# google/telluride_decoding

Hardware: AMD Instinct MI355X
Metric: TRF-fit samples/sec (higher is better)
Workload: dtype f32 (every product as 3 float16 products of a 2-piece split on the f16 MFMA, f32 accumulate, f64 slab sums; f64 solve)

## Files before the change

telluride_decoding_amd/csrc/lag_targets.hip:

```cpp
#include <cstdlib>
#include <cstring>

#include "lag_common.h"

namespace {

constexpr int kWaveStrip = 512;

template <int E, int NI>
__global__ __launch_bounds__(kThreads) void lagcov_wave_kernel(LagParams p, double* __restrict__ part64,
                                                              double* __restrict__ csum,
                                                              double* __restrict__ ysum) {
  constexpr int P = 32;
  constexpr int NY = NI > 0 ? NI : 1;
  constexpr int kRowsMax = ((kWaveStrip + 2 * E - 2) / E) * E;
  __shared__ float ylds[kThreads / 64][kRowsMax * NY];
  const int tid = threadIdx.x, lane = tid & 63;
  const int wave = __builtin_amdgcn_readfirstlane(tid >> 6);
  long long id = blockIdx.x * (long long)(kThreads / 64) + wave;
  if (id >= (long long)p.n_work * p.n_cbt) return;
  const int cbt = (int)(id % p.n_cbt);
  const int wi = (int)(id / p.n_cbt);
  const LagWork w = p.works[wi];
  const int len = (int)(w.u_end - w.u_begin);
// ... 206 lines not shown
      if (!kHalf) slab[(size_t)k * p.ca_pad * p.cb_pad + c0 + 1] = big1[r];
    }
  }
  if (g == 0 && csum) {
    csum[(size_t)slab_i * p.cb_pad + c0] = cs0;
    if (!kHalf) csum[(size_t)slab_i * p.cb_pad + c0 + 1] = cs1;
  }
}

template <bool kVec2, bool kHalf = false>
__global__ __launch_bounds__(kThreads) void lagcov_targets_mfma_kernel(LagParams p,
                                                                       double* __restrict__ part64,
                                                                       double* csum, double* ysum,
                                                                       unsigned* maxtab) {
  constexpr int E = 32, P = kTgtPrefetch, kPad = 32, kRowsBody = 2 * kTgtBody;
  constexpr int kBodiesMax = (kTgtStrip + E - 1 + kRowsBody - 1) / kRowsBody;
  __shared__ float ya[kPad + kBodiesMax * kRowsBody];
  __shared__ double comb[3][16][64];
  const int tid = threadIdx.x, lane = tid & 63;
  const int wave = __builtin_amdgcn_readfirstlane(tid >> 6);
  const int n_win = p.n_groups;
  const int slot = (int)(blockIdx.x >> 3);
  const int item = (slot / n_win) * 8 + (int)(blockIdx.x & 7);
  if (item >= p.n_work * p.n_cbt) return;
  const int cbt = item % p.n_cbt;
  const int wi = item / p.n_cbt;
  const LagWork w = p.works[wi];
  const int e_lo = 32 * (slot % n_win);
  p.e_min += e_lo;
  if (e_lo) { csum = nullptr; ysum = nullptr; maxtab = nullptr; }
  const TgtStrip ts = tgt_strip(p, w);
  const int slab_i = wi;
  tgt_stage_targets(p, w, ts.len, ts.n_body, kPad, ya, tid);
  __syncthreads();
  if (cbt == 0 && ysum && wave == 0) {
    double sy = 0.0;
    for (int t = lane; t < ts.len; t += 64) sy += (double)ya[kPad + t];
#pragma unroll
    for (int off = 32; off > 0; off >>= 1) sy += __shfl_down(sy, off, 64);
    if (lane == 0) ysum[slab_i] = sy;
  }

  const int n = lane & 31, g = lane >> 5;
  const int c0 = kHalf ? cbt * 64 + n : cbt * 64 + 2 * n;
  const bool ok0 = c0 < p.cb, ok1 = !kHalf && c0 + 1 < p.cb;
  const int off0 = ok0 ? c0 : 0, off1 = ok1 ? c0 + 1 : off0;
  int b0 = wave, nb = 0;
  while (b0 < ts.n_body && !tgt_body_fast(ts, b0)) b0 += 4;
  for (int b = b0; b < ts.n_body && tgt_body_fast(ts, b); b += 4) ++nb;

  f32x16 acc0, acc1;
  double big0[16], big1[16];
#pragma unroll
  for (int r = 0; r < 16; ++r) { acc0[r] = 0.f; acc1[r] = 0.f; big0[r] = 0.0; big1[r] = 0.0; }
  double cs0 = 0.0, cs1 = 0.0;
  float mx0 = 0.f, mx1 = 0.f;
  const float* yp = ya + kPad + g - n;
  if (nb > 0) {
    float xr[P][2];
    auto load_step = [&](const float* bp, int s, float& x0, float& x1) {
      if (kHalf) {
        x0 = bp[s * 2 * ts.ldb32]; x1 = 0.f;
      } else if (kVec2) {
        const float2 v = *reinterpret_cast<const float2*>(bp + s * 2 * ts.ldb32);
        x0 = v.x; x1 = v.y;
      } else {
        x0 = bp[s * 2 * ts.ldb32]; x1 = bp[s * 2 * ts.ldb32 + off1 - off0];
      }
    };
    {
      const float* bp = ts.strip + (b0 * kRowsBody + g - ts.r_lo) * ts.ldb32 + off0;
#pragma unroll
      for (int k = 0; k < P; ++k) load_step(bp, k, xr[k][0], xr[k][1]);
    }
    for (int it = 0; it < nb; ++it) {
      const int b = b0 + 4 * it;
      const float* bp = ts.strip + ((b + 4) * kRowsBody + g - ts.r_lo) * ts.ldb32 + off0;
      float c0s = 0.f, c1s = 0.f;
#pragma unroll
      for (int s = 0; s < kTgtBody; ++s) {
        const float x0 = xr[s % P][0], x1 = xr[s % P][1];
        c0s += x0; c1s += x1;
        mx0 = fmaxf(mx0, fabsf(x0)); mx1 = fmaxf(mx1, fabsf(x1));
        const float a = yp[(b * kTgtBody + s) * 2];
        acc0 = __builtin_amdgcn_mfma_f32_32x32x2f32(a, x0, acc0, 0, 0, 0);
        if (!kHalf) acc1 = __builtin_amdgcn_mfma_f32_32x32x2f32(a, x1, acc1, 0, 0, 0);
        load_step(bp, s, xr[s % P][0], xr[s % P][1]);
      }
      cs0 += (double)c0s;
      cs1 += (double)c1s;
#pragma unroll
      for (int r = 0; r < 16; ++r) {
        big0[r] += (double)acc0[r]; acc0[r] = 0.f;
        if (!kHalf) { big1[r] += (double)acc1[r]; acc1[r] = 0.f; }
      }
    }
  }
  for (int b = wave; b < ts.n_body; b += 4) {
    if (tgt_body_fast(ts, b)) continue;
    float c0s = 0.f, c1s = 0.f;
    float xe[kTgtBody][2];
#pragma unroll
    for (int s = 0; s < kTgtBody; ++s) {
      const int r = (b * kTgtBody + s) * 2 + g;
      const int rc = min(max(r, ts.r_lo), ts.r_hi) - ts.r_lo;
      const float* rowp = ts.strip + rc * ts.ldb32;
      if (kHalf) {
        xe[s][0] = rowp[off0]; xe[s][1] = 0.f;
      } else if (kVec2) {
        const float2 v = *reinterpret_cast<const float2*>(rowp + off0);
        xe[s][0] = v.x; xe[s][1] = v.y;
      } else {
        xe[s][0] = rowp[off0]; xe[s][1] = rowp[off1];
      }
    }
#pragma unroll
    for (int s = 0; s < kTgtBody; ++s) {
      const int r = (b * kTgtBody + s) * 2 + g;
      const float m = (r >= ts.r_lo && (long long)r <= ts.last) ? 1.f : 0.f;
      const float x0 = xe[s][0] * m, x1 = xe[s][1] * m;
      mx0 = fmaxf(mx0, fabsf(x0)); mx1 = fmaxf(mx1, fabsf(x1));
      const float in = (r >= ts.t_lo && r < ts.t_hi) ? 1.f : 0.f;
      c0s = fmaf(in, x0, c0s); c1s = fmaf(in, x1, c1s);
      const float a = yp[(b * kTgtBody + s) * 2];
      acc0 = __builtin_amdgcn_mfma_f32_32x32x2f32(a, x0, acc0, 0, 0, 0);
      if (!kHalf) acc1 = __builtin_amdgcn_mfma_f32_32x32x2f32(a, x1, acc1, 0, 0, 0);
    }
    cs0 += (double)c0s;
    cs1 += (double)c1s;
#pragma unroll
    for (int r = 0; r < 16; ++r) {
      big0[r] += (double)acc0[r]; acc0[r] = 0.f;
      if (!kHalf) { big1[r] += (double)acc1[r]; acc1[r] = 0.f; }
    }
  }
  tgt_combine_store<kHalf>(p, part64, csum, maxtab, comb, slab_i, e_lo, c0, ok0, ok1, big0, big1, cs0, cs1,
                           mx0, mx1);
}

constexpr int kTgtBodiesMax = (kTgtStrip + 31 + 31) / 32;
constexpr int kTgtImage = (32 + kTgtBodiesMax * 32) / 2 + 8;

__device__ __forceinline__ int tgt_scale_exp(unsigned max_bits) {
  if (max_bits == 0 || td_chan_not_finite(max_bits)) return 0;
  return 15 - __builtin_amdgcn_frexp_expf(__uint_as_float(max_bits));
}

__device__ __forceinline__ void tgt_split2(float x0, float x1, unsigned& h, unsigned& l) {
  h = td_pack_f16(x0, x1);
  const td_f16x2 hv = __builtin_bit_cast(td_f16x2, h);
  l = td_pack_f16(__builtin_fmaf((float)hv[0], -1.f, x0), __builtin_fmaf((float)hv[1], -1.f, x1));
}

template <class Refill>
__device__ __forceinline__ void tgt_split_body(float (&x)[kTgtBody][2], unsigned mb0, unsigned mb1,
                                               const unsigned* ah, const unsigned* al, int ky, bool y_bad,
                                               double (&big0)[16], double (&big1)[16], Refill refill) {
  mb0 = max(mb0, (unsigned)__shfl_xor((int)mb0, 32, 64));
  mb1 = max(mb1, (unsigned)__shfl_xor((int)mb1, 32, 64));
  const int k0 = tgt_scale_exp(mb0), k1 = tgt_scale_exp(mb1);
  td_u32x4 h0[2], l0[2], h1[2], l1[2];
#pragma unroll
  for (int ks = 0; ks < 2; ++ks)
#pragma unroll
    for (int j = 0; j < 4; ++j) {
      const int s = 8 * ks + 2 * j;
      unsigned h, l;
      tgt_split2(ldexpf(x[s][0], k0), ldexpf(x[s + 1][0], k0), h, l);
      h0[ks][j] = h; l0[ks][j] = l;
      tgt_split2(ldexpf(x[s][1], k1), ldexpf(x[s + 1][1], k1), h, l);
      h1[ks][j] = h; l1[ks][j] = l;
      refill(s);
      refill(s + 1);
    }
  __builtin_amdgcn_sched_barrier(0);
  td_f32x16 acc0, acc1;
#pragma unroll
  for (int r = 0; r < 16; ++r) { acc0[r] = 0.f; acc1[r] = 0.f; }
#pragma unroll
  for (int ks = 0; ks < 2; ++ks) {
    const td_u32x4 yh = {ah[4 * ks], ah[4 * ks + 1], ah[4 * ks + 2], ah[4 * ks + 3]};
    const td_u32x4 yl = {al[4 * ks], al[4 * ks + 1], al[4 * ks + 2], al[4 * ks + 3]};
    acc0 = td_mfma_f16(yl, h0[ks], acc0);
    acc1 = td_mfma_f16(yl, h1[ks], acc1);
    acc0 = td_mfma_f16(yh, l0[ks], acc0);
    acc1 = td_mfma_f16(yh, l1[ks], acc1);
    acc0 = td_mfma_f16(yh, h0[ks], acc0);
    acc1 = td_mfma_f16(yh, h1[ks], acc1);
  }
  const double nan = __hiloint2double(0x7ff80000, 0);
  const double f0 = (y_bad || td_chan_not_finite(mb0)) ? nan : __hiloint2double((1023 - k0 - ky) << 20, 0);
  const double f1 = (y_bad || td_chan_not_finite(mb1)) ? nan : __hiloint2double((1023 - k1 - ky) << 20, 0);
#pragma unroll
  for (int r = 0; r < 16; ++r) {
    big0[r] = fma((double)acc0[r], f0, big0[r]);
    big1[r] = fma((double)acc1[r], f1, big1[r]);
  }
}

__global__ __launch_bounds__(kThreads, 2) void lagcov_targets_split_kernel(LagParams p,
                                                                           double* __restrict__ part64,
                                                                           double* csum, double* ysum,
                                                                           unsigned* maxtab) {
  constexpr int kPad = 32, kRowsBody = 2 * kTgtBody;
  __shared__ float ya[kPad + kTgtBodiesMax * kRowsBody];
  __shared__ __attribute__((aligned(16))) _Float16 yimg[2][2][2][kTgtImage];
  __shared__ double comb[3][16][64];
  __shared__ unsigned ymax_w[kThreads / 64];
  const int tid = threadIdx.x, lane = tid & 63;
  const int wave = __builtin_amdgcn_readfirstlane(tid >> 6);
  const int item = (int)blockIdx.x;
  if (item >= p.n_work * p.n_cbt) return;
  const int cbt = item % p.n_cbt;
  const int wi = item / p.n_cbt;
  const LagWork w = p.works[wi];
  const TgtStrip ts = tgt_strip(p, w);
  const int n = lane & 31, g = lane >> 5;
  const int c0 = cbt * 64 + 2 * n;
  const bool ok0 = c0 < p.cb, ok1 = c0 + 1 < p.cb;
  const int off0 = ok0 ? c0 : 0;
  const int dg = g - n;
  const unsigned* ah = reinterpret_cast<const unsigned*>(&yimg[0][dg & 1][(dg >> 1) & 1][0]) + 8 + (dg >> 2);
  const unsigned* al = reinterpret_cast<const unsigned*>(&yimg[1][dg & 1][(dg >> 1) & 1][0]) + 8 + (dg >> 2);
  int b0 = wave, nb = 0;
  while (b0 < ts.n_body && !tgt_body_fast(ts, b0)) b0 += 4;
  for (int b = b0; b < ts.n_body && tgt_body_fast(ts, b); b += 4) ++nb;

  const long long rows_here = ts.last - ts.r_lo + 1;
  const long long rows_need = (long long)ts.n_body * kRowsBody;
  const unsigned buf_bytes =
      nb > 0 ? (unsigned)(((rows_here < rows_need ? rows_here : rows_need) - 1) * ts.ldb32 + p.cb) * 4u : 0u;
  const __amdgpu_buffer_rsrc_t rs =
      __builtin_amdgcn_make_buffer_rsrc(const_cast<float*>(ts.strip), 0, buf_bytes, 0x00020000);
  const unsigned voff = (unsigned)(g * ts.ldb32 + off0) * 4u;
  float xa[kTgtBody][2], xb[kTgtBody][2];
  auto load_step = [&](float (&xr)[kTgtBody][2], unsigned body_off, int s) {
    const td_f32x2 v = __builtin_bit_cast(
        td_f32x2, __builtin_amdgcn_raw_buffer_load_b64(rs, voff, body_off + (unsigned)(s * 2 * ts.ldb32) * 4u, 0));
    xr[s][0] = v[0]; xr[s][1] = v[1];
  };
  const int b_last = b0 + 4 * (nb - 1);
  auto body_off = [&](int b) { return (unsigned)(((b < b_last ? b : b_last) * kRowsBody - ts.r_lo) * ts.ldb32) * 4u; };
  if (nb > 0) {
    const unsigned bo0 = body_off(b0), bo1 = body_off(b0 + 4);
#pragma unroll
    for (int s = 0; s < kTgtBody; ++s) load_step(xa, bo0, s);
#pragma unroll
    for (int s = 0; s < kTgtBody; ++s) load_step(xb, bo1, s);
  }
  const int n_y = kPad + ts.n_body * kRowsBody;
  tgt_stage_targets(p, w, ts.len, ts.n_body, kPad, ya, tid);
  __syncthreads();
  {
    unsigned ym = 0u;
    for (int t = tid; t < n_y; t += kThreads) ym = max(ym, __float_as_uint(ya[t]) & 0x7fffffffu);
#pragma unroll
    for (int off = 32; off > 0; off >>= 1) ym = max(ym, (unsigned)__shfl_xor((int)ym, off, 64));
    if (lane == 0) ymax_w[wave] = ym;
  }
  if (cbt == 0 && ysum && wave == 0) {
    double sy = 0.0;
    for (int t = lane; t < ts.len; t += 64) sy += (double)ya[kPad + t];
#pragma unroll
    for (int off = 32; off > 0; off >>= 1) sy += __shfl_down(sy, off, 64);
    if (lane == 0) ysum[wi] = sy;
  }
  __syncthreads();
  const unsigned ymax = max(max(ymax_w[0], ymax_w[1]), max(ymax_w[2], ymax_w[3]));
  const bool y_bad = td_chan_not_finite(ymax);
  const int ky = tgt_scale_exp(ymax);
  for (int t = tid; t < n_y / 2; t += kThreads) {
#pragma unroll
    for (int q = 0; q < 2; ++q) {
      const float v = ldexpf(ya[2 * t + q], ky);
      const _Float16 hv = (_Float16)v;
      const _Float16 lv = (_Float16)(v - (float)hv);
      yimg[0][q][0][t] = hv;
      yimg[1][q][0][t] = lv;
      if (t > 0) { yimg[0][q][1][t - 1] = hv; yimg[1][q][1][t - 1] = lv; }
    }
  }
  __syncthreads();

  double big0[16], big1[16];
#pragma unroll
  for (int r = 0; r < 16; ++r) { big0[r] = 0.0; big1[r] = 0.0; }
  double cs0 = 0.0, cs1 = 0.0;
  float mx0 = 0.f, mx1 = 0.f;
  if (nb > 0) {
    auto pass = [&](float (&xr)[kTgtBody][2], int b) {
      const unsigned bo = body_off(b + 8);
      float c0s = 0.f, c1s = 0.f, m0 = 0.f, m1 = 0.f;
#pragma unroll
      for (int s = 0; s < kTgtBody; ++s) {
        c0s += xr[s][0]; c1s += xr[s][1];
        m0 = fmaxf(m0, fabsf(xr[s][0])); m1 = fmaxf(m1, fabsf(xr[s][1]));
      }
      cs0 += (double)c0s;
      cs1 += (double)c1s;
      mx0 = fmaxf(mx0, m0); mx1 = fmaxf(mx1, m1);
      const unsigned mb0 = fabsf(c0s) <= 3.402823466e38f ? __float_as_uint(m0) : 0x7fc00000u;
      const unsigned mb1 = fabsf(c1s) <= 3.402823466e38f ? __float_as_uint(m1) : 0x7fc00000u;
      tgt_split_body(xr, mb0, mb1, ah + 8 * b, al + 8 * b, ky, y_bad, big0, big1,
                     [&](int s) { load_step(xr, bo, s); });
    };
    for (int it = 0; it + 1 < nb; it += 2) {
      pass(xa, b0 + 4 * it);
      pass(xb, b0 + 4 * it + 4);
    }
    if (nb & 1) pass(xa, b0 + 4 * (nb - 1));
  }
  for (int b = wave; b < ts.n_body; b += 4) {
    if (tgt_body_fast(ts, b)) continue;
    float xe[kTgtBody][2];
#pragma unroll
    for (int s = 0; s < kTgtBody; ++s) {
      const int r = (b * kTgtBody + s) * 2 + g;
      const int rc = min(max(r, ts.r_lo), ts.r_hi) - ts.r_lo;
      const float2 v = *reinterpret_cast<const float2*>(ts.strip + rc * ts.ldb32 + off0);
      xe[s][0] = v.x; xe[s][1] = v.y;
    }
    float c0s = 0.f, c1s = 0.f;
    unsigned mb0 = 0u, mb1 = 0u;
#pragma unroll
    for (int s = 0; s < kTgtBody; ++s) {
      const int r = (b * kTgtBody + s) * 2 + g;
      const bool there = r >= ts.r_lo && (long long)r <= ts.last;
      xe[s][0] = there ? xe[s][0] : 0.f;
      xe[s][1] = there ? xe[s][1] : 0.f;
      mx0 = fmaxf(mx0, fabsf(xe[s][0])); mx1 = fmaxf(mx1, fabsf(xe[s][1]));
      mb0 = max(mb0, __float_as_uint(xe[s][0]) & 0x7fffffffu);
      mb1 = max(mb1, __float_as_uint(xe[s][1]) & 0x7fffffffu);
      const float in = (r >= ts.t_lo && r < ts.t_hi) ? 1.f : 0.f;
      c0s = fmaf(in, xe[s][0], c0s); c1s = fmaf(in, xe[s][1], c1s);
    }
    cs0 += (double)c0s;
    cs1 += (double)c1s;
    tgt_split_body(xe, mb0, mb1, ah + 8 * b, al + 8 * b, ky, y_bad, big0, big1, [](int) {});
  }
  tgt_combine_store<false>(p, part64, csum, maxtab, comb, wi, 0, c0, ok0, ok1, big0, big1, cs0, cs1, mx0, mx1);
}

__global__ __launch_bounds__(1024) void colsum_file_reduce_kernel(
    const double* __restrict__ csum, int cb_pad, int cb, const int* __restrict__ file_work0,
    double* __restrict__ out) {
  __shared__ double part[16][64];
  const int f = blockIdx.x, j = blockIdx.y * 64 + (threadIdx.x & 63), q = threadIdx.x >> 6;
  double s0 = 0.0, s1 = 0.0;
  if (j < cb) {
    int wk = file_work0[f] + q;
    const int end = file_work0[f + 1];
    for (; wk + 16 < end; wk += 32) {
      s0 += csum[(size_t)wk * cb_pad + j];
      s1 += csum[(size_t)(wk + 16) * cb_pad + j];
    }
    if (wk < end) s0 += csum[(size_t)wk * cb_pad + j];
  }
  part[q][threadIdx.x & 63] = s0 + s1;
  __syncthreads();
  if (q == 0 && j < cb) {
    double t = 0.0;
#pragma unroll
    for (int k = 0; k < 16; ++k) t += part[k][threadIdx.x];
    out[(size_t)f * cb + j] = t;
  }
}

__global__ __launch_bounds__(256) void ysum_reduce_kernel(const double* __restrict__ ysum, int n_work,
                                                          int ni, double* __restrict__ sy,
                                                          int accumulate) {
  __shared__ double red[256];
  const int i = blockIdx.x;
  double s = 0.0;
  for (int wk = threadIdx.x; wk < n_work; wk += 256) s += ysum[(size_t)wk * ni + i];
  red[threadIdx.x] = s;
  __syncthreads();
  for (int off = 128; off > 0; off >>= 1) {
    if ((int)threadIdx.x < off) red[threadIdx.x] += red[threadIdx.x + off];
    __syncthreads();
  }
  if (threadIdx.x == 0) sy[i] = accumulate ? sy[i] + red[0] : red[0];
}

}

int td_lagcov_targets_plan(td_handle* h, const float* y, int64_t ldy, int d, const float* b,
                           int64_t ldb, int cb, const std::vector<LagSeg>& segs, int e_min,
                           int e_count, TargetsPlan* plan, bool any_lag_window) {
  plan->handled = false;
  plan->scratch_bytes = 0;
  plan->works.clear();
  plan->seg_work0.clear();
  if (any_lag_window) {
    if (d != 1 || e_count > 32 * 8) return TD_OK;
  } else {
    if (d > 4 || e_min > 0 || e_min + e_count - 1 < 0) return TD_OK;
    if (d > 0 ? (e_count > 32 * 8 || (e_count > 32 && e_min < -31)) : -e_min > 31) return TD_OK;
  }
  plan->handled = true;
  plan->lag_window = any_lag_window;
  const int n_segs = (int)segs.size();
  plan->d = d; plan->cb = cb; plan->e_count = e_count; plan->n_segs = n_segs;
  const int ni = d > 0 ? 1 : 0;
  const int slabs_per_strip = 1;
  long long total = 0;
  for (const LagSeg& sg : segs) total += sg.u_end > sg.u_begin ? sg.u_end - sg.u_begin : 0;
  const int cus = h->cu_count > 0 ? h->cu_count : 256;
  long long t_strip = td_round_up(td_ceil_div(total > 0 ? total : 1, 4 * cus), 32);
  t_strip = t_strip < kTgtStripMin ? kTgtStripMin : (t_strip > kTgtStrip ? kTgtStrip : t_strip);
  const long long n_tiles = td_ceil_div(cb, 64);
  auto strips_at = [&](long long t) {
    long long k = 0;
    for (const LagSeg& sg : segs) k += sg.u_end > sg.u_begin ? td_ceil_div(sg.u_end - sg.u_begin, t) : 1;
    return k;
  };
  while (t_strip < kTgtStrip && strips_at(t_strip) * n_tiles > 4LL * cus) t_strip += 32;
  long long w_strip = td_round_up(td_ceil_div(total > 0 ? total : 1, 8 * cus), 32);
  w_strip = w_strip < 128 ? 128 : (w_strip > kWaveStrip ? kWaveStrip : w_strip);
  plan->seg_work0.assign(n_segs + 1, 0);
  for (int f = 0; f < n_segs; ++f) {
    plan->seg_work0[f] = (int)plan->works.size() * slabs_per_strip;
    std::vector<LagSeg> one(1, segs[f]);
    std::vector<LagWork> ws = split_work(one, ni > 0 ? t_strip : w_strip);
    plan->works.insert(plan->works.end(), ws.begin(), ws.end());
  }
  plan->seg_work0[n_segs] = (int)plan->works.size() * slabs_per_strip;
  plan->n_strips = (int)plan->works.size();
  plan->n_work = plan->n_strips * slabs_per_strip;
  LagParams& p = plan->p;
  p.a = y; p.b = b; p.lda = ldy; p.ldb = ldb; p.ca = d; p.cb = cb; p.a_ones = 0;
  p.e_min = e_min; p.e_count = e_count;
  p.n_groups = 1; p.n_cat = 1; p.n_cbt = (int)td_ceil_div(cb, 64);
  p.e_pad = e_count; p.ca_pad = ni > 0 ? ni : 1; p.cb_pad = p.n_cbt * 64;
  p.n_work = plan->n_work;
  p.lag_g = 8; p.lag_lg = 3; p.partial = nullptr; p.works = nullptr;
  const size_t slab_elems = ni > 0 ? (size_t)p.e_pad * p.ca_pad * p.cb_pad : 0;
  plan->part_bytes = td_round_up(slab_elems * plan->n_work * sizeof(double), 256);
  plan->cs_bytes = td_round_up((size_t)plan->n_work * p.cb_pad * sizeof(double), 256);
  plan->ys_bytes = td_round_up((size_t)plan->n_work * sizeof(double), 256);
  const int cols = d > 0 ? d : 1;
  plan->scratch_bytes = plan->cs_bytes + cols * (plan->part_bytes + plan->ys_bytes);
  return TD_OK;
}

int td_lagcov_targets_launch(td_handle* h, TargetsPlan* plan, void* scratch, double* g_dev,
                             bool accumulate, TargetsOutputs* out) {
  LagParams p = plan->p;
  const int d = plan->d, cb = plan->cb, e_count = plan->e_count, n_work = plan->n_work;
  char* base = reinterpret_cast<char*>(scratch);
  double* csum = reinterpret_cast<double*>(base);
  out->csum = csum; out->n_work = n_work; out->cb_pad = p.cb_pad;
  for (int i = 0; i < 4; ++i) out->ysum[i] = nullptr;
  if (n_work == 0) return TD_OK;
  const void* works_dev = nullptr;
  TD_TRY(td_table_upload(h, plan->works.data(), plan->works.size() * sizeof(LagWork), &works_dev));
  p.works = reinterpret_cast<const LagWork*>(works_dev);
  const int cols = d > 0 ? d : 1;
  if (d == 0) {
    double* ysum = reinterpret_cast<double*>(base + plan->cs_bytes + plan->part_bytes);
    const unsigned blocks = (unsigned)td_ceil_div((int64_t)n_work * p.n_cbt, kThreads / 64);
    if (cb <= 32) {
      int cbp = 1;
      while (cbp < cb) cbp <<= 1;
      hipLaunchKernelGGL(colsum_rows_kernel, dim3(blocks), dim3(kThreads), 0, h->stream, p, csum, cbp);
    } else {
      hipLaunchKernelGGL((lagcov_wave_kernel<32, 0>), dim3(blocks), dim3(kThreads), 0, h->stream, p,
                         nullptr, csum, ysum);
    }
  } else {
    const float* y = p.a;
    const bool vec2 = (p.ldb % 2 == 0) && (cb % 2 == 0) && ((reinterpret_cast<uintptr_t>(p.b) & 7) == 0);
    const int n_win = (int)td_ceil_div(e_count, 32);
    p.n_groups = n_win;
    const dim3 grid((unsigned)(td_ceil_div((int64_t)plan->n_strips * p.n_cbt, 8) * 8 * n_win));
    for (int i = 0; i < cols; ++i) {
      LagParams pi = p;
      pi.a = y + i;
      pi.ca = 1;
      char* col = base + plan->cs_bytes + (size_t)i * (plan->part_bytes + plan->ys_bytes);
      double* part64 = reinterpret_cast<double*>(col);
      double* ysum = reinterpret_cast<double*>(col + plan->part_bytes);
      unsigned* maxtab = i == 0 ? out->maxtab : nullptr;
      if (h->targets_f16 && !plan->lag_window && cb > 32 && vec2 && n_win == 1)
        hipLaunchKernelGGL(lagcov_targets_split_kernel, grid, dim3(kThreads), 0, h->stream, pi, part64, csum,
                           ysum, maxtab);
      else if (cb <= 32)
        hipLaunchKernelGGL((lagcov_targets_mfma_kernel<false, true>), grid, dim3(kThreads), 0, h->stream,
                           pi, part64, csum, ysum, maxtab);
      else if (vec2)
        hipLaunchKernelGGL((lagcov_targets_mfma_kernel<true>), grid, dim3(kThreads), 0, h->stream,
                           pi, part64, csum, ysum, maxtab);
      else
        hipLaunchKernelGGL((lagcov_targets_mfma_kernel<false>), grid, dim3(kThreads), 0, h->stream,
                           pi, part64, csum, ysum, maxtab);
      LagReduceJob& job = out->jobs[i];
      job = LagReduceJob{};
      job.partial = part64; job.is_f64 = 1;
      job.n_work = n_work; job.e_pad = p.e_pad; job.ca_pad = p.ca_pad; job.cb_pad = p.cb_pad;
      job.e_count = e_count; job.ca_eff = 1; job.cb = cb;
      job.g = g_dev + (size_t)i * cb; job.accumulate = accumulate ? 1 : 0; job.ca_dst = d + 1;
      job.ldg = cb; job.mirror = 0;
      out->ysum[i] = ysum;
    }
  }
  TD_HIP(h, hipGetLastError());
  return TD_OK;
}

int td_lagcov_targets(td_handle* h, const float* y, int64_t ldy, int d, const float* b, int64_t ldb,
                      int cb, const std::vector<LagSeg>& segs, int e_min, int e_count,
                      double* g_dev, double* sy_dev, double* colsum_seg_dev, bool* handled, int rows_dst) {
  if (rows_dst <= 0) rows_dst = d + 1;
  TargetsPlan plan;
  TD_TRY(td_lagcov_targets_plan(h, y, ldy, d, b, ldb, cb, segs, e_min, e_count, &plan));
  *handled = plan.handled;
  if (!plan.handled || segs.empty()) return TD_OK;
  const int n_segs = plan.n_segs;
  if (plan.n_work == 0) {
    TD_HIP(h, hipMemsetAsync(colsum_seg_dev, 0, sizeof(double) * n_segs * cb, h->stream));
    return TD_OK;
  }
  void* scratch = nullptr;
  TD_TRY(td_scratch(h, plan.scratch_bytes, &scratch));
  TargetsOutputs out;
  out.maxtab = nullptr;
  TD_TRY(td_lagcov_targets_launch(h, &plan, scratch, g_dev, true, &out));
  for (int i = 0; i < d; ++i) {
    LagReduceJob job = out.jobs[i];
    job.ca_dst = rows_dst;
    TD_TRY(td_lagcov_reduce(h, job));
    if (sy_dev)
      hipLaunchKernelGGL(ysum_reduce_kernel, dim3(1), dim3(256), 0, h->stream, out.ysum[i], job.n_work,
                         1, sy_dev + i, 1);
  }
  const void* seg_dev = nullptr;
  TD_TRY(td_table_upload(h, plan.seg_work0.data(), (n_segs + 1) * sizeof(int), &seg_dev));
  hipLaunchKernelGGL(colsum_file_reduce_kernel, dim3((unsigned)n_segs, (unsigned)plan.p.n_cbt),
                     dim3(1024), 0, h->stream, out.csum, plan.p.cb_pad, cb,
                     reinterpret_cast<const int*>(seg_dev), colsum_seg_dev);
  TD_HIP(h, hipGetLastError());
  return TD_OK;
}

int td_lagcov_column(td_handle* h, const float* y, int64_t ldy, const float* b, int64_t ldb, int cb,
                     const std::vector<LagSeg>& segs, int e_min, int e_count, double* g_dev, int rows_dst) {
  if (rows_dst <= 0) rows_dst = 1;
  if (segs.empty()) return TD_OK;
  for (int k0 = 0; k0 < e_count; k0 += 32 * 8) {
    const int cnt = e_count - k0 < 32 * 8 ? e_count - k0 : 32 * 8;
    TargetsPlan plan;
    TD_TRY(td_lagcov_targets_plan(h, y, ldy, 1, b, ldb, cb, segs, e_min + k0, cnt, &plan, true));
    TD_REQUIRE(h, plan.handled, "lagcov_column: the targets kernel refused the shape");
    if (plan.n_work == 0) continue;
    void* scratch = nullptr;
    TD_TRY(td_scratch(h, plan.scratch_bytes, &scratch));
    TargetsOutputs out;
    out.maxtab = nullptr;
    double* dst = g_dev + (size_t)k0 * cb * rows_dst;
    TD_TRY(td_lagcov_targets_launch(h, &plan, scratch, dst, true, &out));
    LagReduceJob job = out.jobs[0];
    job.ca_dst = rows_dst;
    TD_TRY(td_lagcov_reduce(h, job));
  }
  TD_HIP(h, hipGetLastError());
  return TD_OK;
}
```

telluride_decoding_amd/csrc/td_common.h:

```cpp
#pragma once

#include <hip/hip_runtime.h>

#include <cstdarg>
#include <cstdint>
#include <cstdio>
#include <cstring>
#include <string>
#include <vector>

#include "td_hotpath.h"


constexpr int kChanShards = 16;
constexpr int kChanTab = (kChanShards + 1) * 128;

struct td_handle {
  int device = 0;
  int acc_mode = 0;
  int cu_count = 0;
  bool lds_opt_lagcov = false, lds_opt_virt = false, lds_opt_fir = false, lds_opt_fir_stream = false, lds_opt_proj_stream = false;
  bool lds_opt_online = false, lds_opt_online_cca = false, lds_opt_online_dnn = false, lds_opt_online_calib = false;
  hipStream_t own_stream = nullptr;
  hipStream_t stream = nullptr;
// ... 198 lines not shown
struct LagSeg {
  int64_t a_row0;
  int64_t a_valid;
  int64_t b_row0;
  int64_t b_valid;
  int64_t u_begin;
  int64_t u_end;
};

struct LagWork {
  long long a_row0, a_valid, b_row0, b_valid, u_begin, u_end;
};

struct LagParams {
  const float* a;
  const float* b;
  long long lda, ldb;
  int ca, cb;
  int a_ones;
  const LagWork* works;
  int n_work, n_groups, n_cat, n_cbt;
  int e_min, e_count;
  float* partial;
  int n_part;
  int e_pad, ca_pad, cb_pad;
  int lag_g, lag_lg;
  const unsigned* chan_max;
  unsigned* scale_out = nullptr;
  unsigned* zero_tab = nullptr;
  const struct VirtImage* vimgs = nullptr;
  const struct VirtGroup* vgroups = nullptr;
  const struct VirtSeg* vsegs = nullptr;
  long long slab_elems = 0;
};

struct VirtImage {
  short src[64];
  short shift[64];
  signed char role[64];
  short min_shift, max_shift;
  short any_role1, pad;
};
struct VirtTask {
  signed char mt, nt;
  signed char a_ext;
  signed char kparts;
  short lag0;
  short kq;
  int out_lag;
};
struct VirtGroup {
  int image;
  int pad;
  VirtTask task[8];
};
struct VirtSeg {
  long long seg_begin, seg_end;
  long long u_end_ext;
};
struct VirtPair {
  int slot0, E, da, db;
  short nsa, nsb, wa, wb, col_a, col_b;
};
struct VirtMap {
  VirtPair pair[4][4];
};
__host__ __device__ __forceinline__ long long td_virt_offset(const VirtMap* vm, int e, int i, int j, int* e1_out = nullptr) {
  const VirtPair& P = vm->pair[i >> 5][j >> 5];
  int sb = e / P.db;
  sb = sb < P.nsb - 1 ? sb : P.nsb - 1;
  const int rem = e - sb * P.db;
  int sa = rem / P.da;
  sa = sa < P.nsa - 1 ? sa : P.nsa - 1;
  const int e1 = rem - sa * P.da;
  if (e1_out) *e1_out = e1;
  return ((long long)(P.slot0 + e1) * 32 + P.col_a + sa * P.wa + (i & 31)) * 32 + P.col_b + sb * P.wb + (j & 31);
}

struct LagReduceJob {
  const void* partial;
  int is_f64;
  int n_work, e_pad, ca_pad, cb_pad, e_count, ca_eff, cb;
  double* g;
  int accumulate, ca_dst, ldg;
  int mirror;
  const unsigned* scale_a;
  const unsigned* scale_b;
  const struct VirtMap* vmap = nullptr;
  long long slab_elems = 0;
};
int td_lagcov_reduce(td_handle* h, const LagReduceJob& job);

struct LagcovPlan {
  bool force_small = false;
  LagParams p;
  std::vector<LagWork> works;
  bool small = false, few = false, split = false, aligned = false;
  bool narrow = false;
  bool allow_f16 = false;
  bool no_chains = false;
  bool f16 = false;
  std::vector<int> work_seg;
  unsigned* scale_out = nullptr;
  unsigned* zero_tab = nullptr;
  unsigned* tab = nullptr;
  int few_g = 8, ca_eff = 0, cb = 0, e_count = 0;
  int small_lpt = 8;
  long long total = 0, nwg = 0;
  size_t scratch_bytes = 0;
};
int td_lagcov_plan(td_handle* h, const float* a, int64_t lda, int ca, bool a_ones, const float* b,
                   int64_t ldb, int cb, const std::vector<LagSeg>& segs, int e_min, int e_count,
                   LagcovPlan* plan);
int td_lagcov_launch(td_handle* h, LagcovPlan* plan, void* scratch, double* g_dev, bool accumulate,
                     int ldg, int rows_dst, LagReduceJob* job);
struct VirtPlan {
  bool ok = false;
  int c = 0, l = 0, rowdw = 83, n_part = 0, ext = 0;
  bool vec4 = false;
  bool ksplit = false;
  std::vector<VirtImage> images;
  std::vector<VirtGroup> groups;
  VirtMap map;
  std::vector<LagWork> works;
  std::vector<VirtSeg> vsegs;
  long long slab_elems = 0, total = 0, grid = 0;
  size_t scratch_bytes = 0;
};
int td_chan_max(td_handle* h, const float* x, int64_t ldx, int c, long long row0, long long row1, unsigned* tab);
int td_chan_max_works(td_handle* h, const float* x, int64_t ldx, int c, const std::vector<LagWork>& works,
                      unsigned* tab);
int td_lagcov_virt_plan(td_handle* h, const float* x, int64_t ldx, int c, const std::vector<LagSeg>& segs,
                        int l, VirtPlan* plan);
int td_lagcov_virt_launch(td_handle* h, VirtPlan* plan, const float* x, int64_t ldx, void* scratch,
                          const unsigned* tab, double* g_dev, bool accumulate, LagReduceJob* job);
int td_lagcov_virt(td_handle* h, const float* x, int64_t ldx, int c, const std::vector<LagSeg>& segs,
                   int l, double* g_dev, bool accumulate, bool* handled);

int td_chan_tab(td_handle* h, unsigned** tab);

struct TargetsPlan {
  LagParams p;
  std::vector<LagWork> works;
  std::vector<int> seg_work0;
  int d = 0, cb = 0, e_count = 0, n_segs = 0, n_strips = 0, n_work = 0;
  size_t part_bytes = 0, cs_bytes = 0, ys_bytes = 0;
  size_t scratch_bytes = 0;
  bool handled = false;
  bool lag_window = false;
};
int td_lagcov_targets_plan(td_handle* h, const float* y, int64_t ldy, int d, const float* b,
                           int64_t ldb, int cb, const std::vector<LagSeg>& segs, int e_min,
                           int e_count, TargetsPlan* plan, bool any_lag_window = false);
struct TargetsOutputs {
  unsigned* maxtab;
  LagReduceJob jobs[4];
  const double* csum;
  const double* ysum[4];
  int n_work, cb_pad;
};
int td_lagcov_targets_launch(td_handle* h, TargetsPlan* plan, void* scratch, double* g_dev,
                             bool accumulate, TargetsOutputs* out);

struct Narrow16Plan {
  bool ok = false;
  int c = 0, d = 0, pre = 0, l1 = 0, n_lg = 1, lpw = 0;
  std::vector<LagWork> works;
  long long n_part = 0;
  size_t part_bytes = 0, tpart_bytes = 0, cs_bytes = 0, ys_bytes = 0, scratch_bytes = 0;
};
int td_narrow16_plan(td_handle* h, int c, int d, int pre, int l1, int64_t ldx, int64_t ldy,
                     const std::vector<LagSeg>& syx, Narrow16Plan* plan);
int td_narrow16_launch(td_handle* h, Narrow16Plan* plan, const float* x, int64_t ldx, const float* y, int64_t ldy,
                       void* scratch, bool do_main, bool do_targets, double* g_xx, bool acc_main, double* g_xo,
                       bool acc_tgt, LagReduceJob* job, TargetsOutputs* out);

int td_lagcov(td_handle* h, const float* a, int64_t lda, int ca, bool a_ones, const float* b,
              int64_t ldb, int cb, const std::vector<LagSeg>& segs, int e_min, int e_count,
              double* g_dev, bool accumulate, int ldg = 0, int rows_dst = 0, bool skinny = false,
              bool allow_f16 = false, unsigned* chan_tab = nullptr);
int td_chan_tab_scratch(td_handle* h, unsigned** tab);
int td_stats_settle(td_handle* h, td_stats* s);
int td_stats_moments_ld(td_handle* h, td_stats* s, double* xtx_dev, int64_t ld_xtx, double* xty_dev,
                        double* x2tx2_dev, double* xtx2_dev, double* sum_x2_dev);
int td_stats_loso_moments(td_handle* h, td_stats* total, td_stats* const* terms, const int* term_begin,
                          const double* signs, int n_folds, const double* mt, int64_t ld, double* out,
                          double* xty_out);
int td_add_reversed_transposed(td_handle* h, const double* src, int e_count, int ca, int cb, double* dst,
                               int ca_dst = 0);
int td_mirror_upper(td_handle* h, double* g_dev, int c, int ld);

int td_lagcov_column(td_handle* h, const float* y, int64_t ldy, const float* b, int64_t ldb, int cb,
                     const std::vector<LagSeg>& segs, int e_min, int e_count, double* g_dev, int rows_dst = 1);
int td_lagcov_targets(td_handle* h, const float* y, int64_t ldy, int d, const float* b, int64_t ldb,
                      int cb, const std::vector<LagSeg>& segs, int e_min, int e_count,
                      double* g_dev, double* sy_dev, double* colsum_seg_dev, bool* handled, int rows_dst = 0);

struct GramReduceJob {
  const float* partial;
  int n_slabs, n_groups, c1, c2, accumulate;
  double *fxx, *fyy, *gxy, *sx, *sx2;
};

int td_gram(td_handle* h, const float* x, int64_t ldx, int c1, const float* x2, int64_t ldx2, int c2,
            const std::vector<LagSeg>& segs, double* fxx, double* fyy, double* gxy, double* sx,
            double* sx2, bool* handled, bool accumulate = true, double* n_dst = nullptr,
            double n_value = 0.0, GramReduceJob* defer = nullptr);

int td_colsum(td_handle* h, const float* a, int64_t lda, int ca, const std::vector<LagSeg>& segs,
              double* out_dev, bool accumulate);

struct td_chol_state {
  double *a, *rt, *rt8, *sol, *linv, *tol;
  int n, np;
};
size_t td_chol_ws_bytes(int n);
int td_chol_factor(td_handle* h, void* ws, const double* c_dev, int n, const double* bt_dev, int nb,
                   td_chol_state* st, double diag_shift = 0.0, double scale = 1.0);
int td_chol_back(td_handle* h, const td_chol_state* st, const double* ut_dev, int nu, double* xt_dev);
int td_chol_batch_forward(td_handle* h, double* a_dev, double* rt_dev, double* linv_dev, double* tol_dev, int np,
                          int n_real, int nrhs, int batch, int rt_rows);
int td_chol_batch_backward(td_handle* h, double* a_dev, double* rt_dev, double* sol_dev, double* linv_dev, int np,
                           int nrhs, int batch, int rt_rows);
```

Before: 1.212 billion.

## Stream target-split bodies into LDS via direct buffer-to-LDS loads

Replaces the register double-buffered global loads in the targets split kernel with inline-asm buffer_load...lds transfers into a per-wave LDS slot. The slot pool aliases the staged targets and the combine scratch, which cuts LDS use and raises the occupancy hint from 2 to 3 blocks. The split body is restructured to interleave the f16 split and MFMA per k-step instead of refilling registers. A batched target staging loader and a host API exposing the strip-size planner are also added. The single-slot ring forces a full vmcnt wait each body, which can expose load latency, and a new lda limit narrows when the kernel is chosen.

```diff
diff --git a/telluride_decoding_amd/csrc/lag_targets.hip b/telluride_decoding_amd/csrc/lag_targets.hip
--- a/telluride_decoding_amd/csrc/lag_targets.hip
+++ b/telluride_decoding_amd/csrc/lag_targets.hip
@@ -382,41 +382,36 @@
   l = td_pack_f16(__builtin_fmaf((float)hv[0], -1.f, x0), __builtin_fmaf((float)hv[1], -1.f, x1));
 }
 
-template <class Refill>
 __device__ __forceinline__ void tgt_split_body(float (&x)[kTgtBody][2], unsigned mb0, unsigned mb1,
                                                const unsigned* ah, const unsigned* al, int ky, bool y_bad,
-                                               double (&big0)[16], double (&big1)[16], Refill refill) {
+                                               double (&big0)[16], double (&big1)[16]) {
   mb0 = max(mb0, (unsigned)__shfl_xor((int)mb0, 32, 64));
   mb1 = max(mb1, (unsigned)__shfl_xor((int)mb1, 32, 64));
   const int k0 = tgt_scale_exp(mb0), k1 = tgt_scale_exp(mb1);
-  td_u32x4 h0[2], l0[2], h1[2], l1[2];
-#pragma unroll
-  for (int ks = 0; ks < 2; ++ks)
+  td_f32x16 acc0, acc1;
+#pragma unroll
+  for (int r = 0; r < 16; ++r) { acc0[r] = 0.f; acc1[r] = 0.f; }
+#pragma unroll
+  for (int ks = 0; ks < 2; ++ks) {
+    td_u32x4 h0, l0, h1, l1;
 #pragma unroll
     for (int j = 0; j < 4; ++j) {
       const int s = 8 * ks + 2 * j;
       unsigned h, l;
       tgt_split2(ldexpf(x[s][0], k0), ldexpf(x[s + 1][0], k0), h, l);
-      h0[ks][j] = h; l0[ks][j] = l;
+      h0[j] = h; l0[j] = l;
       tgt_split2(ldexpf(x[s][1], k1), ldexpf(x[s + 1][1], k1), h, l);
-      h1[ks][j] = h; l1[ks][j] = l;
-      refill(s);
-      refill(s + 1);
-    }
-  __builtin_amdgcn_sched_barrier(0);
-  td_f32x16 acc0, acc1;
-#pragma unroll
-  for (int r = 0; r < 16; ++r) { acc0[r] = 0.f; acc1[r] = 0.f; }
-#pragma unroll
-  for (int ks = 0; ks < 2; ++ks) {
+      h1[j] = h; l1[j] = l;
+    }
     const td_u32x4 yh = {ah[4 * ks], ah[4 * ks + 1], ah[4 * ks + 2], ah[4 * ks + 3]};
     const td_u32x4 yl = {al[4 * ks], al[4 * ks + 1], al[4 * ks + 2], al[4 * ks + 3]};
-    acc0 = td_mfma_f16(yl, h0[ks], acc0);
-    acc1 = td_mfma_f16(yl, h1[ks], acc1);
-    acc0 = td_mfma_f16(yh, l0[ks], acc0);
-    acc1 = td_mfma_f16(yh, l1[ks], acc1);
-    acc0 = td_mfma_f16(yh, h0[ks], acc0);
-    acc1 = td_mfma_f16(yh, h1[ks], acc1);
+    acc0 = td_mfma_f16(yl, h0, acc0);
+    acc1 = td_mfma_f16(yl, h1, acc1);
+    acc0 = td_mfma_f16(yh, l0, acc0);
+    acc1 = td_mfma_f16(yh, l1, acc1);
+    acc0 = td_mfma_f16(yh, h0, acc0);
+    acc1 = td_mfma_f16(yh, h1, acc1);
+    __builtin_amdgcn_sched_barrier(0);
   }
   const double nan = __hiloint2double(0x7ff80000, 0);
   const double f0 = (y_bad || td_chan_not_finite(mb0)) ? nan : __hiloint2double((1023 - k0 - ky) << 20, 0);
@@ -428,15 +423,65 @@
   }
 }
 
-__global__ __launch_bounds__(kThreads, 2) void lagcov_targets_split_kernel(LagParams p,
+constexpr int kTgtSlotBytes = 32 * 64 * 4;
+constexpr int kTgtRing = 1;
+
+__device__ __forceinline__ void tgt_issue_body(td_u32x4 rs, unsigned lds, unsigned voff, unsigned soff,
+                                               unsigned pitch) {
+  unsigned keep;
+#define TD_TGT_ROW "buffer_load_dword %[v], %[rs], %[so] offen lds\n\ts_add_u32 m0, m0, 0x100\n\ts_add_u32 %[so], %[so], %[pitch]\n\t"
+#define TD_TGT_ROW8 TD_TGT_ROW TD_TGT_ROW TD_TGT_ROW TD_TGT_ROW TD_TGT_ROW TD_TGT_ROW TD_TGT_ROW TD_TGT_ROW
+  asm volatile(
+      "s_mov_b32 %[keep], m0\n\t"
+      "s_mov_b32 m0, %[lds]\n\ts_nop 0\n\t"
+      TD_TGT_ROW8 TD_TGT_ROW8 TD_TGT_ROW8 TD_TGT_ROW8
+      "s_mov_b32 m0, %[keep]"
+      : [keep] "=&s"(keep), [so] "+s"(soff)
+      : [lds] "s"(lds), [rs] "s"(rs), [v] "v"(voff), [pitch] "s"(pitch)
+      : "memory", "scc");
+#undef TD_TGT_ROW8
+#undef TD_TGT_ROW
+}
+
+__device__ __forceinline__ void tgt_stage_targets_batched(const LagParams& p, const LagWork& w, int len,
+                                                          int n_body, int kPad, float* ya, int tid) {
+  constexpr int kLoads = (32 + kTgtBodiesMax * 2 * kTgtBody + kThreads - 1) / kThreads;
+  const int n_y = kPad + n_body * 2 * kTgtBody;
+  const long long u0 = w.u_begin > 0 ? w.u_begin : 0;
+  const long long till = w.u_begin + len < w.a_valid ? w.u_begin + len : w.a_valid;
+  const long long avail = till - u0;
+  const unsigned bytes = avail > 0 ? (unsigned)((avail - 1) * p.lda + 1) * 4u : 0u;
+  const __amdgpu_buffer_rsrc_t rs = __builtin_amdgcn_make_buffer_rsrc(
+      const_cast<float*>(avail > 0 ? p.a + (w.a_row0 + u0) * p.lda : p.a), 0, bytes, 0x00020000);
+  const int first = kPad + (int)(u0 - w.u_begin);
+  const unsigned pitch = (unsigned)p.lda * 4u;
+  float v[kLoads];
+#pragma unroll
+  for (int k = 0; k < kLoads; ++k) {
+    const int t = tid + k * kThreads;
+    const unsigned off = (t >= first && t < n_y) ? (unsigned)(t - first) * pitch : 0x80000000u;
+    v[k] = __builtin_bit_cast(float, __builtin_amdgcn_raw_buffer_load_b32(rs, off, 0, 0));
+  }
+#pragma unroll
+  for (int k = 0; k < kLoads; ++k) {
+    const int t = tid + k * kThreads;
+    if (t < n_y) ya[t] = v[k];
+  }
+}
+
+__global__ __launch_bounds__(kThreads, 3) void lagcov_targets_split_kernel(LagParams p,
                                                                            double* __restrict__ part64,
                                                                            double* csum, double* ysum,
                                                                            unsigned* maxtab) {
-  constexpr int kPad = 32, kRowsBody = 2 * kTgtBody;
-  __shared__ float ya[kPad + kTgtBodiesMax * kRowsBody];
+  constexpr int kPad = 32, kRowsBody = 2 * kTgtBody, kWaves = kThreads / 64;
+  constexpr int kPoolBytes = kWaves * kTgtRing * kTgtSlotBytes;
+  static_assert(kPoolBytes >= (int)sizeof(float) * (kPad + kTgtBodiesMax * kRowsBody), "the staged targets");
+  static_assert(kPoolBytes >= (int)sizeof(double) * 3 * 16 * 64, "the waves' sums");
+  __shared__ __attribute__((aligned(16))) unsigned char pool[kPoolBytes];
   __shared__ __attribute__((aligned(16))) _Float16 yimg[2][2][2][kTgtImage];
-  __shared__ double comb[3][16][64];
-  __shared__ unsigned ymax_w[kThreads / 64];
+  __shared__ unsigned ymax_w[kWaves];
+  float* ya = reinterpret_cast<float*>(pool);
+  double (&comb)[3][16][64] = *reinterpret_cast<double (*)[3][16][64]>(pool);
   const int tid = threadIdx.x, lane = tid & 63;
   const int wave = __builtin_amdgcn_readfirstlane(tid >> 6);
   const int item = (int)blockIdx.x;
@@ -445,41 +490,58 @@
   const int wi = item / p.n_cbt;
   const LagWork w = p.works[wi];
   const TgtStrip ts = tgt_strip(p, w);
-  const int n = lane & 31, g = lane >> 5;
-  const int c0 = cbt * 64 + 2 * n;
-  const bool ok0 = c0 < p.cb, ok1 = c0 + 1 < p.cb;
-  const int off0 = ok0 ? c0 : 0;
-  const int dg = g - n;
-  const unsigned* ah = reinterpret_cast<const unsigned*>(&yimg[0][dg & 1][(dg >> 1) & 1][0]) + 8 + (dg >> 2);
-  const unsigned* al = reinterpret_cast<const unsigned*>(&yimg[1][dg & 1][(dg >> 1) & 1][0]) + 8 + (dg >> 2);
+  struct Lane {
+    int n, g, c0, off0;
+    bool ok0, ok1;
+    const unsigned *ah, *al;
+  };
+  auto lane_of = [&](int ln) {
+    Lane q;
+    q.n = ln & 31; q.g = ln >> 5;
+    q.c0 = cbt * 64 + 2 * q.n;
+    q.ok0 = q.c0 < p.cb; q.ok1 = q.c0 + 1 < p.cb;
+    q.off0 = q.ok0 ? q.c0 : 0;
+    const int dg = q.g - q.n;
+    q.ah = reinterpret_cast<const unsigned*>(&yimg[0][dg & 1][(dg >> 1) & 1][0]) + 8 + (dg >> 2);
+    q.al = reinterpret_cast<const unsigned*>(&yimg[1][dg & 1][(dg >> 1) & 1][0]) + 8 + (dg >> 2);
+    return q;
+  };
+  const Lane ln = lane_of(lane);
+  const int n = ln.n, g = ln.g;
   int b0 = wave, nb = 0;
   while (b0 < ts.n_body && !tgt_body_fast(ts, b0)) b0 += 4;
   for (int b = b0; b < ts.n_body && tgt_body_fast(ts, b); b += 4) ++nb;
+  b0 = __builtin_amdgcn_readfirstlane(b0);
+  nb = __builtin_amdgcn_readfirstlane(nb);
 
   const long long rows_here = ts.last - ts.r_lo + 1;
   const long long rows_need = (long long)ts.n_body * kRowsBody;
+  const long long rows_desc = rows_here < rows_need ? rows_here : rows_need;
   const unsigned buf_bytes =
-      nb > 0 ? (unsigned)(((rows_here < rows_need ? rows_here : rows_need) - 1) * ts.ldb32 + p.cb) * 4u : 0u;
-  const __amdgpu_buffer_rsrc_t rs =
+      rows_desc > 0 ? (unsigned)((rows_desc - 1) * ts.ldb32 + p.cb) * 4u : 0u;
+  const __amdgpu_buffer_rsrc_t rs_edge =
       __builtin_amdgcn_make_buffer_rsrc(const_cast<float*>(ts.strip), 0, buf_bytes, 0x00020000);
-  const unsigned voff = (unsigned)(g * ts.ldb32 + off0) * 4u;
-  float xa[kTgtBody][2], xb[kTgtBody][2];
-  auto load_step = [&](float (&xr)[kTgtBody][2], unsigned body_off, int s) {
-    const td_f32x2 v = __builtin_bit_cast(
-        td_f32x2, __builtin_amdgcn_raw_buffer_load_b64(rs, voff, body_off + (unsigned)(s * 2 * ts.ldb32) * 4u, 0));
-    xr[s][0] = v[0]; xr[s][1] = v[1];
+  const unsigned long long xbase = reinterpret_cast<unsigned long long>(ts.strip);
+  td_u32x4 rs;
+  rs[0] = __builtin_amdgcn_readfirstlane((unsigned)xbase);
+  rs[1] = __builtin_amdgcn_readfirstlane((unsigned)(xbase >> 32) & 0xffffu);
+  rs[2] = __builtin_amdgcn_readfirstlane(buf_bytes);
+  rs[3] = 0x00020000u;
+  const int dma_c = cbt * 64 + lane;
+  const unsigned dma_voff = (unsigned)(dma_c < p.cb ? dma_c : p.cb - 1) * 4u;
+  const unsigned pitch = __builtin_amdgcn_readfirstlane((unsigned)ts.ldb32 * 4u);
+  const unsigned slot_lds = __builtin_amdgcn_readfirstlane(
+      (unsigned)(size_t)(__attribute__((address_space(3))) const unsigned char*)pool +
+      (unsigned)(wave * kTgtRing * kTgtSlotBytes));
+  const float* slot = reinterpret_cast<const float*>(pool + wave * kTgtRing * kTgtSlotBytes) + g * 64 + 2 * n;
+  auto issue = [&](int b) {
+    const unsigned soff = __builtin_amdgcn_readfirstlane((unsigned)((b * kRowsBody - ts.r_lo) * ts.ldb32) * 4u);
+    tgt_issue_body(rs, slot_lds, dma_voff, soff, pitch);
   };
-  const int b_last = b0 + 4 * (nb - 1);
-  auto body_off = [&](int b) { return (unsigned)(((b < b_last ? b : b_last) * kRowsBody - ts.r_lo) * ts.ldb32) * 4u; };
-  if (nb > 0) {
-    const unsigned bo0 = body_off(b0), bo1 = body_off(b0 + 4);
-#pragma unroll
-    for (int s = 0; s < kTgtBody; ++s) load_step(xa, bo0, s);
-#pragma unroll
-    for (int s = 0; s < kTgtBody; ++s) load_step(xb, bo1, s);
-  }
   const int n_y = kPad + ts.n_body * kRowsBody;
-  tgt_stage_targets(p, w, ts.len, ts.n_body, kPad, ya, tid);
+  const bool early = nb > 0 && wave * kTgtRing * kTgtSlotBytes >= n_y * (int)sizeof(float);
+  if (early) issue(b0);
+  tgt_stage_targets_batched(p, w, ts.len, ts.n_body, kPad, ya, tid);
   __syncthreads();
   {
     unsigned ym = 0u;
@@ -511,51 +573,58 @@
     }
   }
   __syncthreads();
+  if (nb > 0 && !early) issue(b0);
 
   double big0[16], big1[16];
 #pragma unroll
   for (int r = 0; r < 16; ++r) { big0[r] = 0.0; big1[r] = 0.0; }
   double cs0 = 0.0, cs1 = 0.0;
   float mx0 = 0.f, mx1 = 0.f;
-  if (nb > 0) {
-    auto pass = [&](float (&xr)[kTgtBody][2], int b) {
-      const unsigned bo = body_off(b + 8);
-      float c0s = 0.f, c1s = 0.f, m0 = 0.f, m1 = 0.f;
-#pragma unroll
-      for (int s = 0; s < kTgtBody; ++s) {
-        c0s += xr[s][0]; c1s += xr[s][1];
-        m0 = fmaxf(m0, fabsf(xr[s][0])); m1 = fmaxf(m1, fabsf(xr[s][1]));
-      }
-      cs0 += (double)c0s;
-      cs1 += (double)c1s;
-      mx0 = fmaxf(mx0, m0); mx1 = fmaxf(mx1, m1);
-      const unsigned mb0 = fabsf(c0s) <= 3.402823466e38f ? __float_as_uint(m0) : 0x7fc00000u;
-      const unsigned mb1 = fabsf(c1s) <= 3.402823466e38f ? __float_as_uint(m1) : 0x7fc00000u;
-      tgt_split_body(xr, mb0, mb1, ah + 8 * b, al + 8 * b, ky, y_bad, big0, big1,
-                     [&](int s) { load_step(xr, bo, s); });
-    };
-    for (int it = 0; it + 1 < nb; it += 2) {
-      pass(xa, b0 + 4 * it);
-      pass(xb, b0 + 4 * it + 4);
-    }
-    if (nb & 1) pass(xa, b0 + 4 * (nb - 1));
-  }
+  for (int it = 0; it < nb; ++it) {
+    const int b = b0 + 4 * it;
+    float xr[kTgtBody][2];
+    asm volatile("s_waitcnt vmcnt(0)" ::: "memory");
+#pragma unroll
+    for (int s = 0; s < kTgtBody; ++s) {
+      const td_f32x2 v = *reinterpret_cast<const td_f32x2*>(slot + s * 128);
+      xr[s][0] = v[0]; xr[s][1] = v[1];
+    }
+    asm volatile("s_waitcnt lgkmcnt(0)" ::: "memory");
+    if (it + 1 < nb) issue(b + 4);
+    float c0s = 0.f, c1s = 0.f, m0 = 0.f, m1 = 0.f;
+#pragma unroll
+    for (int s = 0; s < kTgtBody; ++s) {
+      c0s += xr[s][0]; c1s += xr[s][1];
+      m0 = fmaxf(m0, fabsf(xr[s][0])); m1 = fmaxf(m1, fabsf(xr[s][1]));
+    }
+    cs0 += (double)c0s;
+    cs1 += (double)c1s;
+    mx0 = fmaxf(mx0, m0); mx1 = fmaxf(mx1, m1);
+    const unsigned mb0 = fabsf(c0s) <= 3.402823466e38f ? __float_as_uint(m0) : 0x7fc00000u;
+    const unsigned mb1 = fabsf(c1s) <= 3.402823466e38f ? __float_as_uint(m1) : 0x7fc00000u;
+    tgt_split_body(xr, mb0, mb1, ln.ah + 8 * b, ln.al + 8 * b, ky, y_bad, big0, big1);
+  }
+  int lane_e = lane;
+  asm volatile("" : "+v"(lane_e));
+  const Lane le = lane_of(lane_e);
+  const int last32 = ts.last < -1 ? -1 : (ts.last > (1 << 20) ? (1 << 20) : (int)ts.last);
   for (int b = wave; b < ts.n_body; b += 4) {
     if (tgt_body_fast(ts, b)) continue;
     float xe[kTgtBody][2];
 #pragma unroll
     for (int s = 0; s < kTgtBody; ++s) {
-      const int r = (b * kTgtBody + s) * 2 + g;
+      const int r = (b * kTgtBody + s) * 2 + le.g;
       const int rc = min(max(r, ts.r_lo), ts.r_hi) - ts.r_lo;
-      const float2 v = *reinterpret_cast<const float2*>(ts.strip + rc * ts.ldb32 + off0);
-      xe[s][0] = v.x; xe[s][1] = v.y;
+      const td_f32x2 v = __builtin_bit_cast(
+          td_f32x2, __builtin_amdgcn_raw_buffer_load_b64(rs_edge, (unsigned)(rc * ts.ldb32 + le.off0) * 4u, 0, 0));
+      xe[s][0] = v[0]; xe[s][1] = v[1];
     }
     float c0s = 0.f, c1s = 0.f;
     unsigned mb0 = 0u, mb1 = 0u;
 #pragma unroll
     for (int s = 0; s < kTgtBody; ++s) {
-      const int r = (b * kTgtBody + s) * 2 + g;
-      const bool there = r >= ts.r_lo && (long long)r <= ts.last;
+      const int r = (b * kTgtBody + s) * 2 + le.g;
+      const bool there = r >= ts.r_lo && r <= last32;
       xe[s][0] = there ? xe[s][0] : 0.f;
       xe[s][1] = there ? xe[s][1] : 0.f;
       mx0 = fmaxf(mx0, fabsf(xe[s][0])); mx1 = fmaxf(mx1, fabsf(xe[s][1]));
@@ -566,9 +635,9 @@
     }
     cs0 += (double)c0s;
     cs1 += (double)c1s;
-    tgt_split_body(xe, mb0, mb1, ah + 8 * b, al + 8 * b, ky, y_bad, big0, big1, [](int) {});
-  }
-  tgt_combine_store<false>(p, part64, csum, maxtab, comb, wi, 0, c0, ok0, ok1, big0, big1, cs0, cs1, mx0, mx1);
+    tgt_split_body(xe, mb0, mb1, le.ah + 8 * b, le.al + 8 * b, ky, y_bad, big0, big1);
+  }
+  tgt_combine_store<false>(p, part64, csum, maxtab, comb, wi, 0, le.c0, le.ok0, le.ok1, big0, big1, cs0, cs1, mx0, mx1);
 }
 
 __global__ __launch_bounds__(1024) void colsum_file_reduce_kernel(
@@ -614,6 +683,21 @@
 
 }
 
+static long long tgt_plan_strip(int cus, const std::vector<LagSeg>& segs, int cb) {
+  long long total = 0;
+  for (const LagSeg& sg : segs) total += sg.u_end > sg.u_begin ? sg.u_end - sg.u_begin : 0;
+  long long t_strip = td_round_up(td_ceil_div(total > 0 ? total : 1, 4 * cus), 32);
+  t_strip = t_strip < kTgtStripMin ? kTgtStripMin : (t_strip > kTgtStrip ? kTgtStrip : t_strip);
+  const long long n_tiles = td_ceil_div(cb, 64);
+  auto strips_at = [&](long long t) {
+    long long k = 0;
+    for (const LagSeg& sg : segs) k += sg.u_end > sg.u_begin ? td_ceil_div(sg.u_end - sg.u_begin, t) : 1;
+    return k;
+  };
+  while (t_strip < kTgtStrip && strips_at(t_strip) * n_tiles > 4LL * cus) t_strip += 32;
+  return t_strip;
+}
+
 int td_lagcov_targets_plan(td_handle* h, const float* y, int64_t ldy, int d, const float* b,
                            int64_t ldb, int cb, const std::vector<LagSeg>& segs, int e_min,
                            int e_count, TargetsPlan* plan, bool any_lag_window) {
@@ -633,18 +717,10 @@
   plan->d = d; plan->cb = cb; plan->e_count = e_count; plan->n_segs = n_segs;
   const int ni = d > 0 ? 1 : 0;
   const int slabs_per_strip = 1;
+  const int cus = h->cu_count > 0 ? h->cu_count : 256;
   long long total = 0;
   for (const LagSeg& sg : segs) total += sg.u_end > sg.u_begin ? sg.u_end - sg.u_begin : 0;
-  const int cus = h->cu_count > 0 ? h->cu_count : 256;
-  long long t_strip = td_round_up(td_ceil_div(total > 0 ? total : 1, 4 * cus), 32);
-  t_strip = t_strip < kTgtStripMin ? kTgtStripMin : (t_strip > kTgtStrip ? kTgtStrip : t_strip);
-  const long long n_tiles = td_ceil_div(cb, 64);
-  auto strips_at = [&](long long t) {
-    long long k = 0;
-    for (const LagSeg& sg : segs) k += sg.u_end > sg.u_begin ? td_ceil_div(sg.u_end - sg.u_begin, t) : 1;
-    return k;
-  };
-  while (t_strip < kTgtStrip && strips_at(t_strip) * n_tiles > 4LL * cus) t_strip += 32;
+  const long long t_strip = tgt_plan_strip(cus, segs, cb);
   long long w_strip = td_round_up(td_ceil_div(total > 0 ? total : 1, 8 * cus), 32);
   w_strip = w_strip < 128 ? 128 : (w_strip > kWaveStrip ? kWaveStrip : w_strip);
   plan->seg_work0.assign(n_segs + 1, 0);
@@ -711,7 +787,7 @@
       double* part64 = reinterpret_cast<double*>(col);
       double* ysum = reinterpret_cast<double*>(col + plan->part_bytes);
       unsigned* maxtab = i == 0 ? out->maxtab : nullptr;
-      if (h->targets_f16 && !plan->lag_window && cb > 32 && vec2 && n_win == 1)
+      if (h->targets_f16 && !plan->lag_window && cb > 32 && vec2 && n_win == 1 && pi.lda <= 65536)
         hipLaunchKernelGGL(lagcov_targets_split_kernel, grid, dim3(kThreads), 0, h->stream, pi, part64, csum,
                            ysum, maxtab);
       else if (cb <= 32)
@@ -795,3 +871,17 @@
   TD_HIP(h, hipGetLastError());
   return TD_OK;
 }
+
+extern "C" int td_targets_strip_rows(td_handle* h, const int64_t* rows_host, int num_files, int channels,
+                                     int64_t* strip_rows_out) {
+  if (!h) return td_fail(nullptr, TD_ERR_INVALID, "td_targets_strip_rows: NULL handle");
+  TD_REQUIRE(h, rows_host && strip_rows_out && num_files > 0 && channels > 0, "td_targets_strip_rows: bad arguments");
+  std::vector<LagSeg> segs(num_files);
+  for (int f = 0; f < num_files; ++f) {
+    segs[f] = LagSeg{};
+    segs[f].u_begin = 0;
+    segs[f].u_end = rows_host[f];
+  }
+  *strip_rows_out = tgt_plan_strip(h->cu_count > 0 ? h->cu_count : 256, segs, channels);
+  return TD_OK;
+}
diff --git a/telluride_decoding_amd/csrc/td_common.h b/telluride_decoding_amd/csrc/td_common.h
--- a/telluride_decoding_amd/csrc/td_common.h
+++ b/telluride_decoding_amd/csrc/td_common.h
@@ -374,6 +374,8 @@
 int td_lagcov_targets_plan(td_handle* h, const float* y, int64_t ldy, int d, const float* b,
                            int64_t ldb, int cb, const std::vector<LagSeg>& segs, int e_min,
                            int e_count, TargetsPlan* plan, bool any_lag_window = false);
+extern "C" int td_targets_strip_rows(td_handle* h, const int64_t* rows_host, int num_files, int channels,
+                                     int64_t* strip_rows_out);
 struct TargetsOutputs {
   unsigned* maxtab;
   LagReduceJob jobs[4];
```

Result: no change. 1.213 billion, median of 5 (+0.0%).
